# BichenWuUCB/squeezeDet

Hardware: NVIDIA H100
Metric: images/sec (1242x375, b=20) (higher is better)
Workload: dtype f32 (3xTF32 wgmma, fp32 accumulate)

## Files before the change

squeezedet_b200/csrc/conv_tc.cu:

```cuda
#include <cuda.h>
#include <cuda_runtime.h>
#include <stdint.h>
#include <stdlib.h>
#include <string.h>

#include <vector>

#include "common.cuh"
#include "conv_tc.cuh"

namespace sqdet {
namespace {

constexpr int TILE_M = 128;
constexpr int NUM_THREADS = 256;
constexpr int STAGES = 3;
constexpr int MAX_CHUNKS = 32;
constexpr int FT_W = 16, FQ_W = FT_W + 2, FQ_P = 10 * FQ_W;

enum TcMode { TC_ROWS, TC_GATHER, TC_HALO, TC_FIRE };

struct TcChunk {
  int ksize, pad_t, pad_l;
  int nk;
  int ncount;
  int y_off;
  int p_off;
  long long w_off;
};

struct TcParams {
  CUtensorMap amap, amap1;
  const float* x;
  float* y;
  const float* w;
  const float* bias;
  const float* scale;
  const float* shift;
  int B, H, W, Cin, Ho, Wo, stride, relu, y_cstride;
  long long M;
  int tiles_w, tiles_h;
  int nchunks;
  TcChunk chunks[MAX_CHUNKS];
};

__device__ __forceinline__ uint32_t smem_u32(const void* p) {
  return static_cast<uint32_t>(__cvta_generic_to_shared(p));
}
__device__ __forceinline__ void cp_async4(uint32_t dst, const void* src, bool valid) {
  asm volatile("cp.async.ca.shared.global [%0], [%1], 4, %2;" ::"r"(dst), "l"(src),
               "r"(valid ? 4 : 0)
               : "memory");
}
__device__ __forceinline__ void cp_async_arrive(uint64_t* bar) {
  asm volatile("cp.async.mbarrier.arrive.noinc.shared::cta.b64 [%0];" ::"r"(smem_u32(bar)) : "memory");
}

__device__ __forceinline__ void mbar_init(uint64_t* bar, int count) {
  asm volatile("mbarrier.init.shared::cta.b64 [%0], %1;" ::"r"(smem_u32(bar)), "r"(count) : "memory");
}
__device__ __forceinline__ void mbar_init_fence() {
  asm volatile("fence.mbarrier_init.release.cluster;\n\tfence.proxy.async.shared::cta;" ::: "memory");
}
__device__ __forceinline__ void mbar_arrive(uint64_t* bar) {
  asm volatile("mbarrier.arrive.shared::cta.b64 _, [%0];" ::"r"(smem_u32(bar)) : "memory");
}
__device__ __forceinline__ void mbar_expect_tx(uint64_t* bar, uint32_t bytes) {
  asm volatile("mbarrier.arrive.expect_tx.shared::cta.b64 _, [%0], %1;" ::"r"(smem_u32(bar)),
               "r"(bytes)
               : "memory");
}
__device__ __forceinline__ void mbar_wait(uint64_t* bar, uint32_t parity) {
  asm volatile(
      "{\n\t.reg .pred done;\n\t"
      "WAIT_%=:\n\t"
      "mbarrier.try_wait.parity.shared::cta.b64 done, [%0], %1;\n\t"
      "@!done bra WAIT_%=;\n\t}" ::"r"(smem_u32(bar)),
      "r"(parity)
      : "memory");
}

__device__ __forceinline__ void ring_init(uint64_t* full, uint64_t* empty, int full_count) {
  for (int s = 0; s < STAGES; ++s) {
    mbar_init(&full[s], full_count);
    mbar_init(&empty[s], NUM_THREADS / 32);
  }
  mbar_init_fence();
}
__device__ __forceinline__ int ring_acquire(uint64_t* empty, int j) {
  const int s = j % STAGES;
  if (j >= STAGES) mbar_wait(&empty[s], (j / STAGES & 1) ^ 1);
  return s;
}
__device__ __forceinline__ int ring_wait_full(uint64_t* full, int j) {
  const int s = j % STAGES;
  mbar_wait(&full[s], j / STAGES & 1);
  return s;
}
__device__ __forceinline__ void ring_release(uint64_t* empty, int j) {
  __syncwarp();
  if ((threadIdx.x & 31) == 0) mbar_arrive(&empty[j % STAGES]);
}

__device__ __forceinline__ void bulk_load(uint32_t dst, const void* src, uint32_t bytes, uint64_t* bar) {
  asm volatile(
      "cp.async.bulk.shared::cluster.global.mbarrier::complete_tx::bytes [%0], [%1], %2, [%3];" ::"r"(dst),
      "l"(src), "r"(bytes), "r"(smem_u32(bar))
      : "memory");
}
__device__ __forceinline__ void tma_load(uint32_t dst, const CUtensorMap* map, int c0, int c1, uint64_t* bar) {
  asm volatile(
      "cp.async.bulk.tensor.2d.shared::cluster.global.tile.mbarrier::complete_tx::bytes "
      "[%0], [%1, {%2, %3}], [%4];" ::"r"(dst),
      "l"(map), "r"(c0), "r"(c1), "r"(smem_u32(bar))
      : "memory");
}
__device__ __forceinline__ void tma_load(uint32_t dst, const CUtensorMap* map, int c0, int c1, int c2,
                                         int c3, uint64_t* bar) {
  asm volatile(
      "cp.async.bulk.tensor.4d.shared::cluster.global.tile.mbarrier::complete_tx::bytes "
      "[%0], [%1, {%2, %3, %4, %5}], [%6];" ::"r"(dst),
      "l"(map), "r"(c0), "r"(c1), "r"(c2), "r"(c3), "r"(smem_u32(bar))
      : "memory");
}
__device__ __forceinline__ void cluster_sync() {
  asm volatile("barrier.cluster.arrive.release.aligned;\n\tbarrier.cluster.wait.acquire.aligned;" ::: "memory");
}
__device__ __forceinline__ float4 ld_cluster_f4(uint32_t addr, int rank) {
  float4 v;
  asm volatile(
      "{\n\t.reg .b32 ra;\n\t"
      "mapa.shared::cluster.u32 ra, %4, %5;\n\t"
      "ld.shared::cluster.v4.f32 {%0, %1, %2, %3}, [ra];\n\t}"
      : "=f"(v.x), "=f"(v.y), "=f"(v.z), "=f"(v.w)
      : "r"(addr), "r"(rank)
      : "memory");
  return v;
}
__device__ __forceinline__ void wgmma_fence() { asm volatile("wgmma.fence.sync.aligned;" ::: "memory"); }
__device__ __forceinline__ void wgmma_commit() {
  asm volatile("wgmma.commit_group.sync.aligned;" ::: "memory");
}
template <int N>
__device__ __forceinline__ void wgmma_wait() {
  asm volatile("wgmma.wait_group.sync.aligned %0;" ::"n"(N) : "memory");
}
__device__ __forceinline__ void fence_operand(float& r) { asm volatile("" : "+f"(r)::"memory"); }
__device__ __forceinline__ void fence_operand(uint32_t& r) { asm volatile("" : "+r"(r)::"memory"); }

__device__ __forceinline__ uint64_t make_desc(uint32_t addr, uint32_t sbo) {
  return (uint64_t)((addr & 0x3FFFFu) >> 4) | ((uint64_t)(128 >> 4) << 16) |
         ((uint64_t)(sbo >> 4) << 32);
}

__device__ __forceinline__ float rn_tf32(float x) {
  return __uint_as_float((__float_as_uint(x) + 0x1000u) & 0xFFFFE000u);
}

template <int N>
struct Mma;
template <>
struct Mma<16> {
  static __device__ __forceinline__ void run(float (&d)[8], const uint32_t (&a)[4], uint64_t b,
                                             int acc) {
    asm volatile(
        "{\n\t.reg .pred p;\n\tsetp.ne.b32 p, %13, 0;\n\t"
        "wgmma.mma_async.sync.aligned.m64n16k8.f32.tf32.tf32 "
        "{%0, %1, %2, %3, %4, %5, %6, %7}, {%8, %9, %10, %11}, %12, p, 1, 1;\n\t}"
        : "+f"(d[0]), "+f"(d[1]), "+f"(d[2]), "+f"(d[3]), "+f"(d[4]), "+f"(d[5]), "+f"(d[6]),
          "+f"(d[7])
        : "r"(a[0]), "r"(a[1]), "r"(a[2]), "r"(a[3]), "l"(b), "r"(acc));
  }
};
template <>
struct Mma<32> {
  static __device__ __forceinline__ void run(float (&d)[16], const uint32_t (&a)[4], uint64_t b,
                                             int acc) {
    asm volatile(
        "{\n\t.reg .pred p;\n\tsetp.ne.b32 p, %21, 0;\n\t"
        "wgmma.mma_async.sync.aligned.m64n32k8.f32.tf32.tf32 "
        "{%0, %1, %2, %3, %4, %5, %6, %7, %8, %9, %10, %11, %12, %13, %14, %15}, "
        "{%16, %17, %18, %19}, %20, p, 1, 1;\n\t}"
        : "+f"(d[0]), "+f"(d[1]), "+f"(d[2]), "+f"(d[3]), "+f"(d[4]), "+f"(d[5]), "+f"(d[6]),
          "+f"(d[7]), "+f"(d[8]), "+f"(d[9]), "+f"(d[10]), "+f"(d[11]), "+f"(d[12]), "+f"(d[13]),
          "+f"(d[14]), "+f"(d[15])
        : "r"(a[0]), "r"(a[1]), "r"(a[2]), "r"(a[3]), "l"(b), "r"(acc));
  }
};
template <>
struct Mma<64> {
  static __device__ __forceinline__ void run(float (&d)[32], const uint32_t (&a)[4], uint64_t b,
                                             int acc) {
    asm volatile(
        "{\n\t.reg .pred p;\n\tsetp.ne.b32 p, %37, 0;\n\t"
        "wgmma.mma_async.sync.aligned.m64n64k8.f32.tf32.tf32 "
        "{%0, %1, %2, %3, %4, %5, %6, %7, %8, %9, %10, %11, %12, %13, %14, %15, "
        "%16, %17, %18, %19, %20, %21, %22, %23, %24, %25, %26, %27, %28, %29, %30, %31}, "
        "{%32, %33, %34, %35}, %36, p, 1, 1;\n\t}"
        : "+f"(d[0]), "+f"(d[1]), "+f"(d[2]), "+f"(d[3]), "+f"(d[4]), "+f"(d[5]), "+f"(d[6]),
          "+f"(d[7]), "+f"(d[8]), "+f"(d[9]), "+f"(d[10]), "+f"(d[11]), "+f"(d[12]), "+f"(d[13]),
          "+f"(d[14]), "+f"(d[15]), "+f"(d[16]), "+f"(d[17]), "+f"(d[18]), "+f"(d[19]),
          "+f"(d[20]), "+f"(d[21]), "+f"(d[22]), "+f"(d[23]), "+f"(d[24]), "+f"(d[25]),
          "+f"(d[26]), "+f"(d[27]), "+f"(d[28]), "+f"(d[29]), "+f"(d[30]), "+f"(d[31])
        : "r"(a[0]), "r"(a[1]), "r"(a[2]), "r"(a[3]), "l"(b), "r"(acc));
  }
};
template <>
struct Mma<72> {
  static __device__ __forceinline__ void run(float (&d)[36], const uint32_t (&a)[4], uint64_t b,
                                             int acc) {
    asm volatile(
        "{\n\t.reg .pred p;\n\tsetp.ne.b32 p, %41, 0;\n\t"
        "wgmma.mma_async.sync.aligned.m64n72k8.f32.tf32.tf32 "
        "{%0, %1, %2, %3, %4, %5, %6, %7, %8, %9, %10, %11, %12, %13, %14, %15, "
        "%16, %17, %18, %19, %20, %21, %22, %23, %24, %25, %26, %27, %28, %29, %30, %31, "
        "%32, %33, %34, %35}, "
        "{%36, %37, %38, %39}, %40, p, 1, 1;\n\t}"
        : "+f"(d[0]), "+f"(d[1]), "+f"(d[2]), "+f"(d[3]), "+f"(d[4]), "+f"(d[5]), "+f"(d[6]),
          "+f"(d[7]), "+f"(d[8]), "+f"(d[9]), "+f"(d[10]), "+f"(d[11]), "+f"(d[12]), "+f"(d[13]),
          "+f"(d[14]), "+f"(d[15]), "+f"(d[16]), "+f"(d[17]), "+f"(d[18]), "+f"(d[19]),
          "+f"(d[20]), "+f"(d[21]), "+f"(d[22]), "+f"(d[23]), "+f"(d[24]), "+f"(d[25]),
          "+f"(d[26]), "+f"(d[27]), "+f"(d[28]), "+f"(d[29]), "+f"(d[30]), "+f"(d[31]),
          "+f"(d[32]), "+f"(d[33]), "+f"(d[34]), "+f"(d[35])
        : "r"(a[0]), "r"(a[1]), "r"(a[2]), "r"(a[3]), "l"(b), "r"(acc));
  }
};

__host__ __device__ constexpr int halo_rows(int KC) {
  return (FQ_P * KC * 4 + 1023) / 1024 * 1024 / (KC * 4);
}
static_assert(2 * halo_rows(16) <= STAGES * TILE_M && 2 * halo_rows(32) <= STAGES * TILE_M,
              "two halo tiles fit in the A ring");
constexpr size_t conv_smem_bytes(int NT, int KC) {
  return 1024 + (size_t)STAGES * (2 * NT * KC + TILE_M * KC) * sizeof(float) + 2 * STAGES * sizeof(uint64_t);
}

__device__ __forceinline__ void split(const float (&v)[4], uint32_t (&ahi)[4], uint32_t (&alo)[4]) {
#pragma unroll
  for (int i = 0; i < 4; ++i) {
    const float hi = rn_tf32(v[i]);
    ahi[i] = __float_as_uint(hi);
    alo[i] = __float_as_uint(rn_tf32(v[i] - hi));
  }
}

__device__ __forceinline__ void load_split(const float* a0, const float* a1, int ks, int t,
                                           uint32_t (&ahi)[4], uint32_t (&alo)[4]) {
  split({a0[ks * 8 + t], a1[ks * 8 + t], a0[ks * 8 + t + 4], a1[ks * 8 + t + 4]}, ahi, alo);
}

template <int KC>
__device__ __forceinline__ int swz(int p) {
  return KC == 32 ? (p & 7) : ((p >> 1) & 3);
}
template <int KC>
__device__ __forceinline__ void load_split_swz(const float* tile, int p, int ks, int t,
                                               uint32_t (&ahi)[4], uint32_t (&alo)[4]) {
  const float* a0 = tile + p * KC + t;
  const float* a1 = a0 + 8 * KC;
  const int j0 = (2 * ks ^ swz<KC>(p)) * 4, j1 = ((2 * ks + 1) ^ swz<KC>(p)) * 4;
  split({a0[j0], a1[j0], a0[j1], a1[j1]}, ahi, alo);
}

template <int NT, int KC>
__device__ __forceinline__ void mma_step(float (&acc)[NT / 2], const uint32_t (&ahi)[4],
                                         const uint32_t (&alo)[4], uint32_t bhi, int ks) {
  constexpr uint32_t SBO = (KC / 4) * 128;
  const uint32_t blo = bhi + NT * KC * 4;
  const uint64_t dhi = make_desc(bhi + ks * 256, SBO), dlo = make_desc(blo + ks * 256, SBO);
#pragma unroll
  for (int i = 0; i < NT / 2; ++i) fence_operand(acc[i]);
  wgmma_fence();
  Mma<NT>::run(acc, alo, dhi, 0);
  Mma<NT>::run(acc, ahi, dlo, 1);
  Mma<NT>::run(acc, ahi, dhi, 1);
  wgmma_commit();
}

template <int N>
__device__ __forceinline__ void flush(float (&acc)[N], float (&sum)[N], uint32_t (&ahi)[4],
                                      uint32_t (&alo)[4]) {
#pragma unroll
  for (int i = 0; i < 4; ++i) fence_operand(ahi[i]), fence_operand(alo[i]);
#pragma unroll
  for (int i = 0; i < N; ++i) {
    fence_operand(acc[i]);
    sum[i] += acc[i];
  }
}

template <int NT, int KC, bool PIPE = true, typename LoadA>
__device__ __forceinline__ void mma_chunk(LoadA load_a, uint32_t bhi, float (&acc)[2][NT / 2],
                                          float (&sum)[NT / 2]) {
  constexpr int KSTEPS = KC / 8;
  uint32_t ahi[2][4], alo[2][4];
  if constexpr (!PIPE) {
#pragma unroll
    for (int ks = 0; ks < KSTEPS; ++ks) {
      load_a(ks, ahi[0], alo[0]);
      mma_step<NT, KC>(acc[0], ahi[0], alo[0], bhi, ks);
      wgmma_wait<0>();
      flush(acc[0], sum, ahi[0], alo[0]);
    }
  } else {
#pragma unroll
    for (int ks = 0; ks < KSTEPS; ++ks) {
      const int cur = ks & 1;
      load_a(ks, ahi[cur], alo[cur]);
      mma_step<NT, KC>(acc[cur], ahi[cur], alo[cur], bhi, ks);
      if (ks > 0) {
        wgmma_wait<1>();
        flush(acc[cur ^ 1], sum, ahi[cur ^ 1], alo[cur ^ 1]);
      }
    }
    constexpr int last = (KSTEPS - 1) & 1;
    wgmma_wait<0>();
    flush(acc[last], sum, ahi[last], alo[last]);
  }
}

struct HaloTile {
  int n, oy0, ox0;
};
__device__ __forceinline__ HaloTile halo_tile(int tiles_w, int tiles_h) {
  const int tx = blockIdx.x % tiles_w, rest = blockIdx.x / tiles_w;
  return {rest / tiles_h, rest % tiles_h * 8, tx * FT_W};
}

__device__ __forceinline__ float finish(const TcParams& p, const TcChunk& ch, int c, float v) {
  if (p.bias) v += p.bias[ch.p_off + c];
  if (p.scale) v = v * p.scale[ch.p_off + c] + p.shift[ch.p_off + c];
  if (p.relu) v = fmaxf(v, 0.f);
  return v;
}

template <typename Value>
__device__ __forceinline__ void store_pair(float* yrow, int c, int ncount, bool pair, Value value) {
  if (pair && c + 1 < ncount) {
    *reinterpret_cast<float2*>(yrow + c) = make_float2(value(c), value(c + 1));
  } else {
    if (c < ncount) yrow[c] = value(c);
    if (c + 1 < ncount) yrow[c + 1] = value(c + 1);
  }
}
__device__ __forceinline__ bool rows_pair_aligned(const TcParams& p, const TcChunk& ch) {
  return ((p.y_cstride | ch.y_off) & 1) == 0 && (reinterpret_cast<uintptr_t>(p.y) & 7) == 0;
}

template <int NT, int KC, int MODE, bool KSPLIT = false>
__global__ void __launch_bounds__(NUM_THREADS, 2)
conv_tc_kernel(const __grid_constant__ TcParams p) {
  static_assert(!KSPLIT || MODE == TC_HALO, "the K split walks halo-mode channel chunks");
  constexpr int NACC = NT / 2;
  constexpr int WST = 2 * NT * KC;
  constexpr uint32_t W_BYTES = WST * 4, TILE_BYTES = TILE_M * KC * 4, HALO_BYTES = FQ_P * KC * 4;
  constexpr int HROWS = halo_rows(KC);
  extern __shared__ __align__(16) uint8_t smem_raw[];
  float* const smem = reinterpret_cast<float*>(smem_raw + ((1024 - (smem_u32(smem_raw) & 1023)) & 1023));
  float* const sa = smem + STAGES * WST;
  uint64_t* const full = reinterpret_cast<uint64_t*>(sa + STAGES * TILE_M * KC);
  uint64_t* const empty = full + STAGES;

  const TcChunk& ch = p.chunks[blockIdx.y];
  const int tid = threadIdx.x;
  const int wg = tid >> 7, wq = (tid >> 5) & 3, lane = tid & 31, g = lane >> 2, t = lane & 3;
  const float* wch = p.w + ch.w_off;
  int k0 = 0, nk = ch.nk;
  const int taps = ch.ksize * ch.ksize;
  if (KSPLIT) {
    const int nc = ch.nk / taps, S = gridDim.z, z = blockIdx.z;
    k0 = z * nc / S * taps;
    nk = (z + 1) * nc / S * taps - k0;
    wch += (size_t)k0 * WST;
  }

  if (tid == 0) ring_init(full, empty, MODE == TC_GATHER ? NUM_THREADS + 1 : 1);
  __syncthreads();

  const long long m0 = (long long)blockIdx.x * TILE_M;

  auto gather_stage = [&](int kk, int s) {
    const int lp = tid >> 1, lh = tid & 1;
    const long long lm = m0 + lp;
    const bool lvalid = lm < p.M;
    int ln = 0, liy0 = 0, lix0 = 0;
    if (lvalid) {
      const int hw = p.Ho * p.Wo;
      ln = (int)(lm / hw);
      const int r = (int)(lm - (long long)ln * hw);
      liy0 = (r / p.Wo) * p.stride - ch.pad_t;
      lix0 = (r % p.Wo) * p.stride - ch.pad_l;
    }
    const float* xn = p.x + (size_t)ln * p.H * p.W * p.Cin;
    float* const arow = sa + (s * TILE_M + lp) * KC;
#pragma unroll
    for (int j = 0; j < KC / 2; ++j) {
      const int col = lh * (KC / 2) + j, k = kk * KC + col;
      const int tap = k / p.Cin, c = k - tap * p.Cin;
      const int iy = liy0 + tap / ch.ksize, ix = lix0 + tap % ch.ksize;
      const bool ok = lvalid && tap < taps && iy >= 0 && iy < p.H && ix >= 0 && ix < p.W;
      cp_async4(smem_u32(arow + ((col >> 2 ^ swz<KC>(lp)) << 2) + (col & 3)),
                ok ? xn + ((iy * p.W + ix) * p.Cin + c) : p.x, ok);
    }
    cp_async_arrive(&full[s]);
  };

  auto load_stage = [&](int j) {
    if (MODE != TC_GATHER && tid != 0) return;
    const int s = ring_acquire(empty, j);
    if (MODE == TC_GATHER) gather_stage(j, s);
    if (tid != 0) return;
    uint32_t bytes = W_BYTES;
    if (MODE == TC_ROWS) {
      bytes += TILE_BYTES;
      mbar_expect_tx(&full[s], bytes);
      tma_load(smem_u32(sa + s * TILE_M * KC), &p.amap, j * KC, (int)m0, &full[s]);
    } else if (MODE == TC_HALO) {
      const HaloTile tl = halo_tile(p.tiles_w, p.tiles_h);
      if (taps == 1) {
        bytes += TILE_BYTES;
        mbar_expect_tx(&full[s], bytes);
        tma_load(smem_u32(sa + s * TILE_M * KC), &p.amap1, (k0 + j) * KC, tl.ox0, tl.oy0, tl.n, &full[s]);
      } else if (j % 9 == 0) {
        bytes += HALO_BYTES;
        mbar_expect_tx(&full[s], bytes);
        tma_load(smem_u32(sa + (j / 9 & 1) * HROWS * KC), &p.amap, (k0 + j) / 9 * KC, tl.ox0 - 1,
                 tl.oy0 - 1, tl.n, &full[s]);
      } else {
        mbar_expect_tx(&full[s], bytes);
      }
    } else {
      mbar_expect_tx(&full[s], bytes);
    }
    bulk_load(smem_u32(smem + s * WST), wch + (size_t)j * WST, W_BYTES, &full[s]);
  };

#pragma unroll 1
  for (int j = 0; j < STAGES - 1 && j < nk; ++j) load_stage(j);

  const int arow0 = wg * 64 + wq * 16 + g;
  const int r = wg * 4 + wq;
  float acc[2][NACC], sum[NACC];
#pragma unroll
  for (int i = 0; i < NACC; ++i) acc[0][i] = acc[1][i] = sum[i] = 0.f;

  for (int kk = 0; kk < nk; ++kk) {
    if (kk + STAGES - 1 < nk) load_stage(kk + STAGES - 1);
    const int s = ring_wait_full(full, kk);

    const float* tile = sa + s * TILE_M * KC;
    int prow = arow0;
    if (MODE == TC_HALO && taps > 1) {
      const int c = kk / 9, tap = kk - c * 9;
      tile = sa + (c & 1) * HROWS * KC;
      prow = (r + tap / 3) * FQ_W + g + tap % 3;
    }
    mma_chunk<NT, KC, NT != 72>(
        [&](int ks, uint32_t(&ahi)[4], uint32_t(&alo)[4]) { load_split_swz<KC>(tile, prow, ks, t, ahi, alo); },
        smem_u32(smem + s * WST), acc, sum);
    ring_release(empty, kk);
  }

  if constexpr (KSPLIT) {
    static_assert(TILE_M * NT <= STAGES * (WST + TILE_M * KC), "the partial tile fits in the ring");
    float* const part = smem;
    __syncthreads();
#pragma unroll
    for (int h = 0; h < 2; ++h)
#pragma unroll
      for (int j = 0; j < NT / 8; ++j)
        *reinterpret_cast<float2*>(part + (arow0 + 8 * h) * NT + 8 * j + 2 * t) =
            make_float2(sum[4 * j + 2 * h], sum[4 * j + 2 * h + 1]);
    cluster_sync();
    constexpr int G = TILE_M * NT / 4;
    const int S = gridDim.z, z = blockIdx.z;
    const HaloTile tl = halo_tile(p.tiles_w, p.tiles_h);
    for (int i = z * G / S + tid; i < (z + 1) * G / S; i += NUM_THREADS) {
      const uint32_t at = smem_u32(part + 4 * i);
      float4 v = ld_cluster_f4(at, 0);
      for (int q = 1; q < S; ++q) {
        const float4 u = ld_cluster_f4(at, q);
        v.x += u.x, v.y += u.y, v.z += u.z, v.w += u.w;
      }
      const int px = 4 * i / NT, c0 = 4 * i % NT;
      const int oy = tl.oy0 + px / FT_W, ox = tl.ox0 + px % FT_W;
      if (oy >= p.Ho || ox >= p.Wo) continue;
      float* yrow = p.y + (((size_t)tl.n * p.Ho + oy) * p.Wo + ox) * p.y_cstride + ch.y_off;
      const float vs[4] = {v.x, v.y, v.z, v.w};
#pragma unroll
      for (int e = 0; e < 4; ++e)
        if (c0 + e < ch.ncount) yrow[c0 + e] = finish(p, ch, c0 + e, vs[e]);
    }
    cluster_sync();
  } else {
    const bool pair = rows_pair_aligned(p, ch);
#pragma unroll
    for (int h = 0; h < 2; ++h) {
      long long m = m0 + arow0 + 8 * h;
      if (MODE == TC_HALO) {
        const HaloTile tl = halo_tile(p.tiles_w, p.tiles_h);
        const int oy = tl.oy0 + r, ox = tl.ox0 + g + 8 * h;
        if (oy >= p.Ho || ox >= p.Wo) continue;
        m = ((long long)tl.n * p.Ho + oy) * p.Wo + ox;
      } else if (m >= p.M) {
        continue;
      }
      float* yrow = p.y + (size_t)m * p.y_cstride + ch.y_off;
#pragma unroll
      for (int j = 0; j < NT / 8; ++j)
        store_pair(yrow, 8 * j + 2 * t, ch.ncount, pair,
                   [&](int c) { return finish(p, ch, c, sum[4 * j + 2 * h + (c & 1)]); });
    }
  }
}

constexpr int FS = 16;
constexpr int FQ_ROWS = 192;

__host__ __device__ constexpr int fire_stage_floats(int KCI) { return 2 * FS * KCI + FQ_ROWS * KCI; }
constexpr size_t fire_smem_bytes(int KCI) {
  return 1024 + ((size_t)STAGES * fire_stage_floats(KCI) + FQ_ROWS * (FS + 4)) * sizeof(float) +
         2 * STAGES * sizeof(uint64_t);
}

template <int KCI>
__global__ void __launch_bounds__(NUM_THREADS, 2)
fire_tc_kernel(const __grid_constant__ TcParams p) {
  constexpr int QP = FS + 4;
  constexpr int SQW = 2 * FS * KCI;
  constexpr int STAGE = fire_stage_floats(KCI);
  constexpr uint32_t SQW_BYTES = SQW * 4, HALO_BYTES = FQ_P * KCI * 4, EX_BYTES = 2 * 64 * FS * 4;
  static_assert(EX_BYTES <= (SQW + FQ_P * KCI) * 4, "expand tile fits before the zeroed rows");
  static_assert(SQW_BYTES % 1024 == 0 && STAGE * 4 % 1024 == 0, "A tiles keep the swizzle's alignment");
  extern __shared__ __align__(16) uint8_t smem_raw[];
  float* const smem = reinterpret_cast<float*>(smem_raw + ((1024 - (smem_u32(smem_raw) & 1023)) & 1023));
  float* const q = smem + STAGES * STAGE;
  uint64_t* const full = reinterpret_cast<uint64_t*>(q + FQ_ROWS * QP);
  uint64_t* const empty = full + STAGES;

  const int tid = threadIdx.x;
  const int wg = tid >> 7, wq = (tid >> 5) & 3, lane = tid & 31, g = lane >> 2, t = lane & 3;
  const int nks = p.Cin / KCI;
  int total = 0;
#pragma unroll 1
  for (int c = 0; c < p.nchunks; ++c) total += p.chunks[c].nk;
  if (tid == 0) ring_init(full, empty, 1);
  for (int i = tid; i < STAGES * (FQ_ROWS - FQ_P) * KCI; i += NUM_THREADS) {
    const int s = i / ((FQ_ROWS - FQ_P) * KCI);
    smem[s * STAGE + SQW + FQ_P * KCI + i % ((FQ_ROWS - FQ_P) * KCI)] = 0.f;
  }
  __syncthreads();

  auto load_stage = [&](int j) {
    const int s = ring_acquire(empty, j);
    float* const st = smem + s * STAGE;
    if (j < nks) {
      const HaloTile tl = halo_tile(p.tiles_w, p.tiles_h);
      mbar_expect_tx(&full[s], SQW_BYTES + HALO_BYTES);
      tma_load(smem_u32(st + SQW), &p.amap, j * KCI, tl.ox0 - 1, tl.oy0 - 1, tl.n, &full[s]);
      bulk_load(smem_u32(st), p.w + (size_t)j * SQW, SQW_BYTES, &full[s]);
    } else {
      mbar_expect_tx(&full[s], EX_BYTES);
      bulk_load(smem_u32(st), p.w + (size_t)nks * SQW + (size_t)(j - nks) * 2 * 64 * FS, EX_BYTES,
                &full[s]);
    }
  };
  if (tid == 0) {
#pragma unroll 1
    for (int j = 0; j < STAGES - 1 && j < total; ++j) load_stage(j);
  }

  float accq[2][FS / 2], sq[2][FS / 2];
#pragma unroll
  for (int i = 0; i < FS / 2; ++i) accq[0][i] = accq[1][i] = sq[0][i] = sq[1][i] = 0.f;
  const int rb = wq * 16 + g;
  for (int kk = 0; kk < nks; ++kk) {
    if (tid == 0 && kk + STAGES - 1 < total) load_stage(kk + STAGES - 1);
    const float* st = smem + ring_wait_full(full, kk) * STAGE;
    const float* sa = st + SQW;
    if (wg == 0) {
      uint32_t qhi[2][4], qlo[2][4];
#pragma unroll
      for (int j = 0; j < 2 * (KCI / 8); ++j) {
        const int bi = j & 1, ks = j >> 1;
        load_split_swz<KCI>(sa, 128 * bi + rb, ks, t, qhi[bi], qlo[bi]);
        mma_step<FS, KCI>(accq[bi], qhi[bi], qlo[bi], smem_u32(st), ks);
        if (j > 0) {
          wgmma_wait<1>();
          flush(accq[bi ^ 1], sq[bi ^ 1], qhi[bi ^ 1], qlo[bi ^ 1]);
        }
      }
      wgmma_wait<0>();
      flush(accq[1], sq[1], qhi[1], qlo[1]);
    } else {
      mma_chunk<FS, KCI>(
          [&](int ks, uint32_t(&ahi)[4], uint32_t(&alo)[4]) {
            load_split_swz<KCI>(sa, 64 + rb, ks, t, ahi, alo);
          },
          smem_u32(st), accq, sq[0]);
    }
    ring_release(empty, kk);
  }
  {
    const HaloTile tl = halo_tile(p.tiles_w, p.tiles_h);
#pragma unroll
    for (int bi = 0; bi < 2; ++bi) {
      const int b = wg + 2 * bi;
      if (b >= 3) continue;
#pragma unroll
      for (int h = 0; h < 2; ++h) {
        const int row = b * 64 + wq * 16 + g + 8 * h;
        const int iy = tl.oy0 - 1 + row / FQ_W, ix = tl.ox0 - 1 + row % FQ_W;
        const bool ok = row < FQ_P && iy >= 0 && iy < p.H && ix >= 0 && ix < p.W;
#pragma unroll
        for (int j = 0; j < FS / 8; ++j)
#pragma unroll
          for (int e = 0; e < 2; ++e) {
            const int c = 8 * j + 2 * t + e;
            q[row * QP + c] = ok ? fmaxf(sq[bi][4 * j + 2 * h + e] + p.bias[c], 0.f) : 0.f;
          }
      }
    }
  }
  __syncthreads();

  const int r = wg * 4 + wq;
  float acc[2][32], sum[32];
#pragma unroll
  for (int i = 0; i < 32; ++i) acc[0][i] = acc[1][i] = sum[i] = 0.f;
  int c = 1, kk = 0;
  for (int j = nks; j < total; ++j) {
    if (tid == 0 && j + STAGES - 1 < total) load_stage(j + STAGES - 1);
    const int s = ring_wait_full(full, j);
    const TcChunk& ch = p.chunks[c];
    const int dy = ch.nk == 1 ? 1 : kk / 3, dx = ch.nk == 1 ? 1 : kk % 3;
    const int qr = (r + dy) * FQ_W + g + dx;
    mma_chunk<64, FS>(
        [&](int ks, uint32_t(&ahi)[4], uint32_t(&alo)[4]) {
          load_split(q + qr * QP, q + (qr + 8) * QP, ks, t, ahi, alo);
        },
        smem_u32(smem + s * STAGE), acc, sum);
    ring_release(empty, j);
    if (++kk == ch.nk) {
      const HaloTile tl = halo_tile(p.tiles_w, p.tiles_h);
      const int oy = tl.oy0 + r;
      const size_t prow = ((size_t)tl.n * p.H + oy) * p.W;
      const bool pair = rows_pair_aligned(p, ch);
#pragma unroll
      for (int h = 0; h < 2; ++h) {
        const int ox = tl.ox0 + g + 8 * h;
        if (oy >= p.H || ox >= p.W) continue;
        float* yrow = p.y + (prow + ox) * p.y_cstride + ch.y_off;
#pragma unroll
        for (int jn = 0; jn < 8; ++jn)
          store_pair(yrow, 8 * jn + 2 * t, ch.ncount, pair, [&](int col) {
            return fmaxf(sum[4 * jn + 2 * h + (col & 1)] + p.bias[ch.p_off + col], 0.f);
          });
      }
#pragma unroll
      for (int i = 0; i < 32; ++i) sum[i] = 0.f;
      kk = 0;
      ++c;
    }
  }
}

using TcKernel = void (*)(TcParams);

template <int KC, int MODE>
TcKernel conv_tc_instance(int NT) {
  return NT == 64 ? conv_tc_kernel<64, KC, MODE>
         : NT == 32 ? conv_tc_kernel<32, KC, MODE> : conv_tc_kernel<16, KC, MODE>;
}

TcKernel conv_tc_instance(int NT, int KC, int mode) {
  if (NT == 72) return mode == TC_HALO ? conv_tc_kernel<72, 32, TC_HALO> : conv_tc_kernel<72, 32, TC_ROWS>;
  if (mode == TC_GATHER) return conv_tc_instance<32, TC_GATHER>(NT);
  if (mode == TC_HALO)
    return KC == 32 ? conv_tc_instance<32, TC_HALO>(NT) : conv_tc_instance<16, TC_HALO>(NT);
  return KC == 32 ? conv_tc_instance<32, TC_ROWS>(NT) : conv_tc_instance<16, TC_ROWS>(NT);
}

struct PlanGroup {
  ConvGroup conv;
  int NT, KC, cin, chunk0;
};

}

struct TcImpl {
  TcParams prm{};
  int KC = 0;
  int mode = TC_ROWS;
  TcKernel kernel = nullptr;
  int ksplit = 1;
  size_t smem_bytes = 0;
  std::vector<PlanGroup> groups;
  int cout_total = 0;
  float* d_w = nullptr;
  float* d_bias = nullptr;
  float* d_scale = nullptr;
  float* d_shift = nullptr;
  long long w_floats = 0;
  const float* map_x = nullptr;
  int map_n = 0;
};

static inline float host_rn_tf32(float x) {
  uint32_t u;
  memcpy(&u, &x, 4);
  u = (u + 0x1000u) & 0xFFFFE000u;
  float r;
  memcpy(&r, &u, 4);
  return r;
}

static int pick_nt(const std::vector<ConvGroup>& groups, int KC, bool gather) {
  int best = 0;
  long long best_cost = 0;
  const bool head = !gather && KC == 32 && groups.size() == 1 && groups[0].Cout > 64 &&
                    groups[0].Cout <= 72;
  for (int nt : {72, 64, 32, 16}) {
    if (nt == 72 && !head) continue;
    long long chunks = 0;
    for (const auto& g : groups) chunks += (g.Cout + nt - 1) / nt;
    if (chunks > MAX_CHUNKS) continue;
    const long long cost = chunks * (nt + 32);
    if (!best || cost < best_cost) best = nt, best_cost = cost;
  }
  return best;
}

using EncodeTiledFn = CUresult (*)(CUtensorMap*, CUtensorMapDataType, cuuint32_t, void*, const cuuint64_t*,
                                   const cuuint64_t*, const cuuint32_t*, const cuuint32_t*,
                                   CUtensorMapInterleave, CUtensorMapSwizzle, CUtensorMapL2promotion,
                                   CUtensorMapFloatOOBfill);

static int encode_map(CUtensorMap* map, const float* x, int rank, const cuuint64_t* dims,
                      const cuuint32_t* box, int KC) {
  static EncodeTiledFn encode = [] {
    void* fn = nullptr;
    cudaDriverEntryPointQueryResult q;
    if (cudaGetDriverEntryPoint("cuTensorMapEncodeTiled", &fn, cudaEnableDefault, &q) != cudaSuccess ||
        q != cudaDriverEntryPointSuccess)
      fn = nullptr;
    return reinterpret_cast<EncodeTiledFn>(fn);
  }();
  if (!encode) return fail(SQDET_ERR_CUDA, "cuTensorMapEncodeTiled is not available from the driver");
  cuuint64_t strides[3];
  cuuint64_t stride = sizeof(float);
  for (int i = 0; i + 1 < rank; ++i) strides[i] = stride *= dims[i];
  const cuuint32_t elem_strides[4] = {1, 1, 1, 1};
  const CUresult rc = encode(map, CU_TENSOR_MAP_DATA_TYPE_FLOAT32, rank, const_cast<float*>(x), dims, strides,
                             box, elem_strides, CU_TENSOR_MAP_INTERLEAVE_NONE,
                             KC == 32 ? CU_TENSOR_MAP_SWIZZLE_128B : CU_TENSOR_MAP_SWIZZLE_64B,
                             CU_TENSOR_MAP_L2_PROMOTION_L2_128B, CU_TENSOR_MAP_FLOAT_OOB_FILL_NONE);
  if (rc != CUDA_SUCCESS)
    return fail(SQDET_ERR_CUDA, "cuTensorMapEncodeTiled failed (error " + std::to_string((int)rc) + ")");
  return SQDET_OK;
}

static int encode_nhwc_map(CUtensorMap* map, const float* x, int n, int H, int W, int C, int KC,
                           int box_w, int box_h) {
  const cuuint64_t dims[4] = {(cuuint64_t)C, (cuuint64_t)W, (cuuint64_t)H, (cuuint64_t)n};
  const cuuint32_t box[4] = {(cuuint32_t)KC, (cuuint32_t)box_w, (cuuint32_t)box_h, 1};
  return encode_map(map, x, 4, dims, box, KC);
}

static int update_maps(TcImpl* im, const float* x, int n) {
  if (im->mode == TC_GATHER || (im->map_x == x && im->map_n == n)) return SQDET_OK;
  TcParams& p = im->prm;
  im->map_x = nullptr;
  int rc;
  if (im->mode == TC_ROWS) {
    const cuuint64_t dims[2] = {(cuuint64_t)p.Cin, (cuuint64_t)n * p.H * p.W};
    const cuuint32_t box[2] = {(cuuint32_t)im->KC, TILE_M};
    rc = encode_map(&p.amap, x, 2, dims, box, im->KC);
  } else {
    rc = encode_nhwc_map(&p.amap, x, n, p.H, p.W, p.Cin, im->KC, FQ_W, 10);
    if (!rc && im->mode == TC_HALO) rc = encode_nhwc_map(&p.amap1, x, n, p.H, p.W, p.Cin, im->KC, FT_W, 8);
  }
  if (rc) return rc;
  im->map_x = x;
  im->map_n = n;
  return SQDET_OK;
}

static long long grid_blocks(const TcImpl* im, int n) {
  const TcParams& p = im->prm;
  if (im->mode == TC_HALO || im->mode == TC_FIRE) return (long long)n * p.tiles_h * p.tiles_w;
  return ((long long)n * p.Ho * p.Wo + TILE_M - 1) / TILE_M;
}

static int plan_common(TcImpl* im, int B, int H, int W, int Cin, int Ho, int Wo, int stride,
                       int pad_t, int pad_l, int relu, bool has_affine, int y_cstride) {
  const bool gather = im->mode == TC_GATHER;
  TcParams& p = im->prm;
  p.B = B; p.H = H; p.W = W; p.Cin = Cin; p.Ho = Ho; p.Wo = Wo; p.stride = stride;
  p.relu = relu; p.y_cstride = y_cstride; p.M = (long long)B * Ho * Wo;
  p.tiles_w = (Wo + FT_W - 1) / FT_W; p.tiles_h = (Ho + 7) / 8;
  if (p.M <= 0 || grid_blocks(im, B) > 0x7fffffffLL) return 0;
  std::vector<int> poffs;
  int poff = 0;
  for (const auto& g : im->groups) poffs.push_back(poff), poff += g.conv.Cout;
  std::vector<size_t> order;
  for (int pass = 0; pass < 2; ++pass)
    for (size_t gi = 0; gi < im->groups.size(); ++gi)
      if ((im->mode == TC_HALO && im->groups[gi].conv.ksize == 3) == (pass == 0)) order.push_back(gi);
  int nch = 0;
  long long woff = 0;
  for (const size_t gi : order) {
    PlanGroup& g = im->groups[gi];
    g.chunk0 = nch;
    const int taps = g.conv.ksize * g.conv.ksize;
    const int nk = gather ? (taps * g.cin + g.KC - 1) / g.KC : taps * (g.cin / g.KC);
    for (int cb = 0; cb < g.conv.Cout; cb += g.NT, ++nch) {
      TcChunk& c = p.chunks[nch];
      c.ksize = g.conv.ksize;
      c.pad_t = gather ? pad_t : g.conv.ksize / 2;
      c.pad_l = gather ? pad_l : g.conv.ksize / 2;
      c.nk = nk;
      c.ncount = g.conv.Cout - cb < g.NT ? g.conv.Cout - cb : g.NT;
      c.y_off = g.conv.y_off + cb;
      c.p_off = poffs[gi] + cb;
      c.w_off = woff;
      woff += (long long)nk * 2 * g.NT * g.KC;
    }
  }
  p.nchunks = nch;
  im->cout_total = poff;
  im->w_floats = woff;
  cudaError_t ce = cudaFuncSetAttribute(im->kernel, cudaFuncAttributeMaxDynamicSharedMemorySize,
                                        (int)im->smem_bytes);
  if (ce != cudaSuccess) return cuda_fail(ce, "cudaFuncSetAttribute(tensor-core kernel)");
  SQ_CUDA(cudaMalloc(&im->d_w, sizeof(float) * (size_t)woff));
  SQ_CUDA(cudaMalloc(&im->d_bias, sizeof(float) * poff));
  SQ_CUDA(cudaMemset(im->d_bias, 0, sizeof(float) * poff));
  if (has_affine) {
    SQ_CUDA(cudaMalloc(&im->d_scale, sizeof(float) * poff));
    SQ_CUDA(cudaMalloc(&im->d_shift, sizeof(float) * poff));
  }
  p.w = im->d_w;
  p.bias = im->d_bias;
  p.scale = im->d_scale;
  p.shift = im->d_shift;
  return 1;
}

static void pack_tiles(const float* w, long long kreal, int cout, int n0, int NT, int KC, int nk,
                       int taps, int cin, float* dst) {
  for (int kk = 0; kk < nk; ++kk) {
    float* hi_t = dst + (size_t)kk * 2 * NT * KC;
    float* lo_t = hi_t + NT * KC;
    const long long k0 = (long long)(kk % taps) * cin + (long long)(kk / taps) * KC;
    for (int n = 0; n < NT; ++n)
      for (int k = 0; k < KC; ++k) {
        const long long kg = k0 + k;
        const float v = (n0 + n < cout && kg < kreal) ? w[kg * cout + n0 + n] : 0.f;
        const float hi = host_rn_tf32(v);
        const size_t at = ((size_t)(n / 8) * (KC / 4) + k / 4) * 32 + (n % 8) * 4 + k % 4;
        hi_t[at] = hi;
        lo_t[at] = host_rn_tf32(v - hi);
      }
  }
}

static void pack_group(const TcImpl* im, const PlanGroup& g, const float* w_hwio, std::vector<float>& packed) {
  const int taps = im->mode == TC_GATHER ? 1 : g.conv.ksize * g.conv.ksize;
  int ci = g.chunk0;
  for (int cb = 0; cb < g.conv.Cout; cb += g.NT, ++ci) {
    const TcChunk& c = im->prm.chunks[ci];
    pack_tiles(w_hwio, (long long)g.conv.ksize * g.conv.ksize * g.cin, g.conv.Cout, cb, g.NT, g.KC,
               c.nk, taps, g.cin, packed.data() + c.w_off);
  }
}

struct ClusterLaunch {
  cudaLaunchAttribute attr;
  cudaLaunchConfig_t cfg;
  ClusterLaunch(dim3 grid, size_t smem, int S, cudaStream_t stream) : attr{}, cfg{} {
    attr.id = cudaLaunchAttributeClusterDimension;
    attr.val.clusterDim.x = attr.val.clusterDim.y = 1;
    attr.val.clusterDim.z = (unsigned)S;
    cfg.gridDim = dim3(grid.x, grid.y, grid.z * S);
    cfg.blockDim = dim3(NUM_THREADS);
    cfg.dynamicSmemBytes = smem;
    cfg.stream = stream;
    cfg.attrs = &attr;
    cfg.numAttrs = 1;
  }
};

constexpr int MAX_KSPLIT = 4;
constexpr int MIN_RANK_CHUNKS = 4;

static int plan_ksplit(TcImpl* im, int forced) {
  const TcKernel split = conv_tc_kernel<72, 32, TC_HALO, true>;
  const int nc = im->prm.chunks[0].nk / 9;
  if (forced < 0 || forced > MAX_KSPLIT || forced > nc)
    return fail(SQDET_ERR_INVALID_ARG, "K split outside [1, min(4, channel chunks)]");
  SQ_CUDA(cudaFuncSetAttribute(split, cudaFuncAttributeMaxDynamicSharedMemorySize, (int)im->smem_bytes));
  int S = forced;
  if (!forced) {
    int dev = 0, sms = 0, per_sm = 0;
    SQ_CUDA(cudaGetDevice(&dev));
    SQ_CUDA(cudaDeviceGetAttribute(&sms, cudaDevAttrMultiProcessorCount, dev));
    SQ_CUDA(cudaOccupancyMaxActiveBlocksPerMultiprocessor(&per_sm, im->kernel, NUM_THREADS, im->smem_bytes));
    const long long ctas = grid_blocks(im, im->prm.B) * im->prm.nchunks;
    S = 1;
    long long best_waves = (ctas + per_sm * sms - 1) / (per_sm * sms);
    for (int s = 2; s <= MAX_KSPLIT && s * MIN_RANK_CHUNKS <= nc; ++s) {
      int clusters = 0;
      const ClusterLaunch l(dim3(1), im->smem_bytes, s, nullptr);
      SQ_CUDA(cudaOccupancyMaxActiveClusters(&clusters, split, &l.cfg));
      if (clusters < 1) continue;
      const long long waves = (ctas + clusters - 1) / clusters;
      if (waves * S < best_waves * s) S = s, best_waves = waves;
    }
  }
  if (S > 1) im->kernel = split;
  im->ksplit = S;
  return 1;
}

bool tc_conv_eligible(int Cin, int Cout, int size, int stride, int padding) {
  if (stride != 1 || padding != SQDET_PAD_SAME || (size != 1 && size != 3)) return false;
  return Cin % 16 == 0 && Cin >= 16 && Cout > 0;
}

int tc_conv_plan(TcConvPlan* plan, int B, int H, int W, int Cin, const std::vector<ConvGroup>& convs,
                 int stride, int padding, int relu, bool has_affine, int y_cstride, int k_split) {
  plan->impl = nullptr;
  const int size = convs[0].ksize;
  const bool gather = convs.size() == 1 && Cin == 3 && size == 3 && (stride == 1 || stride == 2) &&
                      convs[0].Cout > 0;
  if (!gather)
    for (const auto& g : convs)
      if (!tc_conv_eligible(Cin, g.Cout, g.ksize, stride, padding)) return 0;
  const Geom gh = tf_geometry(H, size, stride, padding);
  const Geom gw = tf_geometry(W, size, stride, padding);
  if (gh.out <= 0 || gw.out <= 0) return 0;
  const int KC = (gather || Cin % 32 == 0) ? 32 : 16;
  const int NT = pick_nt(convs, KC, gather);
  if (!NT) return 0;
  int mode = gather ? TC_GATHER : TC_ROWS;
  for (const auto& g : convs)
    if (!gather && g.ksize == 3) mode = TC_HALO;
  TcImpl* im = plan->impl = new TcImpl();
  im->KC = KC;
  im->mode = mode;
  im->kernel = conv_tc_instance(NT, KC, mode);
  im->smem_bytes = conv_smem_bytes(NT, KC);
  for (const auto& g : convs) im->groups.push_back({g, NT, KC, Cin, 0});
  int rc = plan_common(im, B, H, W, Cin, gh.out, gw.out, stride, gh.pad_before, gw.pad_before,
                       relu, has_affine, y_cstride);
  if (rc > 0 && NT == 72 && mode == TC_HALO) {
    rc = plan_ksplit(im, k_split);
  } else if (rc > 0 && k_split > 1) {
    rc = fail(SQDET_ERR_INVALID_ARG, "a K split needs a 72-wide 3x3 tensor-core plan");
  }
  if (rc <= 0) tc_conv_release(plan);
  return rc;
}

int tc_conv_k_split(const TcConvPlan& plan) { return plan.impl ? plan.impl->ksplit : 1; }

int tc_fire_plan(TcConvPlan* plan, int B, int H, int W, int Cin, int S, int E1, int E3) {
  plan->impl = nullptr;
  if (Cin % 16 || Cin < 16 || S != FS || E1 <= 0 || E3 <= 0) return 0;
  if ((E1 + 63) / 64 + (E3 + 63) / 64 > 16) return 0;
  const int KCI = Cin % 32 == 0 ? 32 : 16;
  TcImpl* im = plan->impl = new TcImpl();
  im->KC = KCI;
  im->mode = TC_FIRE;
  im->kernel = KCI == 32 ? fire_tc_kernel<32> : fire_tc_kernel<16>;
  im->smem_bytes = fire_smem_bytes(KCI);
  im->groups = {{{1, FS, 0}, FS, KCI, Cin, 0}, {{1, E1, 0}, 64, FS, FS, 0}, {{3, E3, E1}, 64, FS, FS, 0}};
  const int rc = plan_common(im, B, H, W, Cin, H, W, 1, 0, 0, 1, false, E1 + E3);
  if (rc <= 0) tc_conv_release(plan);
  return rc;
}

int tc_conv_pack_weights(TcConvPlan* plan, const std::vector<const float*>& w_hwio,
                         const std::vector<const float*>& bias) {
  TcImpl* im = plan->impl;
  std::vector<float> packed((size_t)im->w_floats, 0.f);
  for (size_t gi = 0; gi < im->groups.size(); ++gi) pack_group(im, im->groups[gi], w_hwio[gi], packed);
  SQ_CUDA(cudaMemcpy(im->d_w, packed.data(), packed.size() * sizeof(float), cudaMemcpyHostToDevice));
  int off = 0;
  for (size_t gi = 0; gi < im->groups.size(); ++gi) {
    const int n = im->groups[gi].conv.Cout;
    if (bias[gi]) SQ_CUDA(cudaMemcpy(im->d_bias + off, bias[gi], sizeof(float) * n, cudaMemcpyHostToDevice));
    off += n;
  }
  return SQDET_OK;
}

int tc_conv_set_affine(TcConvPlan* plan, const float* scale, const float* shift) {
  TcImpl* im = plan->impl;
  if (!im->d_scale) return fail(SQDET_ERR_STATE, "tc conv planned without an affine epilogue");
  SQ_CUDA(cudaMemcpy(im->d_scale, scale, sizeof(float) * im->cout_total, cudaMemcpyHostToDevice));
  SQ_CUDA(cudaMemcpy(im->d_shift, shift, sizeof(float) * im->cout_total, cudaMemcpyHostToDevice));
  return SQDET_OK;
}

int launch_conv_tc(const TcConvPlan& plan, const float* x_dev, float* y_dev, int n,
                   cudaStream_t stream) {
  TcImpl* im = plan.impl;
  if (n < 1 || n > im->prm.B) return fail(SQDET_ERR_INVALID_ARG, "launch_conv_tc: image count outside [1, B]");
  const int rc = update_maps(im, x_dev, n);
  if (rc) return rc;
  TcParams prm = im->prm;
  prm.x = x_dev;
  prm.y = y_dev;
  prm.B = n;
  prm.M = (long long)n * prm.Ho * prm.Wo;
  const dim3 grid((unsigned)grid_blocks(im, n), im->mode == TC_FIRE ? 1u : (unsigned)prm.nchunks);
  if (im->ksplit > 1) {
    const ClusterLaunch l(grid, im->smem_bytes, im->ksplit, stream);
    SQ_CUDA(cudaLaunchKernelEx(&l.cfg, im->kernel, prm));
  } else {
    im->kernel<<<grid, NUM_THREADS, im->smem_bytes, stream>>>(prm);
  }
  SQ_CHECK_LAUNCH(im->mode == TC_FIRE ? "fire_tc_kernel" : "conv_tc_kernel");
  return SQDET_OK;
}

void tc_conv_release(TcConvPlan* plan) {
  TcImpl* im = plan->impl;
  if (!im) return;
  cudaFree(im->d_w);
  cudaFree(im->d_bias);
  cudaFree(im->d_scale);
  cudaFree(im->d_shift);
  delete im;
  plan->impl = nullptr;
}

int tc_conv_oneshot(TcConvPlan* plan, const std::vector<const float*>& w_hwio_dev,
                    const std::vector<const float*>& bias_dev, const float* scale_dev,
                    const float* shift_dev, const float* x_dev, float* y_dev, cudaStream_t stream) {
  TcImpl* im = plan->impl;
  if (!im) return 1;
  const size_t ng = im->groups.size();
  std::vector<std::vector<float>> w(ng), b(ng);
  std::vector<float> sc, sh;
  std::vector<const float*> w_host(ng), b_host(ng);
  cudaError_t ce = cudaSuccess;
  auto download = [&ce](std::vector<float>& dst, const float* src, size_t n) {
    dst.resize(n);
    if (ce == cudaSuccess) ce = cudaMemcpy(dst.data(), src, n * sizeof(float), cudaMemcpyDeviceToHost);
    return dst.data();
  };
  for (size_t gi = 0; gi < ng; ++gi) {
    const ConvGroup& g = im->groups[gi].conv;
    w_host[gi] = download(w[gi], w_hwio_dev[gi], (size_t)g.ksize * g.ksize * im->groups[gi].cin * g.Cout);
    b_host[gi] = bias_dev[gi] ? download(b[gi], bias_dev[gi], g.Cout) : nullptr;
  }
  if (scale_dev) download(sc, scale_dev, im->cout_total), download(sh, shift_dev, im->cout_total);
  int rc = ce == cudaSuccess ? tc_conv_pack_weights(plan, w_host, b_host)
                             : cuda_fail(ce, "tc_conv_oneshot: parameter download");
  if (!rc && scale_dev) rc = tc_conv_set_affine(plan, sc.data(), sh.data());
  if (!rc) rc = launch_conv_tc(*plan, x_dev, y_dev, im->prm.B, stream);
  ce = cudaStreamSynchronize(stream);
  tc_conv_release(plan);
  if (rc) return rc;
  if (ce != cudaSuccess) return cuda_fail(ce, "tc_conv_oneshot sync");
  return SQDET_OK;
}

}
```

Measured before the change: 4820.

## Pack two 3x3 taps per pipeline stage in halo and fire-expand kernels

For halo-mode convolutions with 16-channel chunks and for the fire expand phase, each ring stage now holds the weights for two taps instead of one. The per-stage barrier waits, releases and bulk-load issues drop to roughly half, and each stage runs longer back-to-back wgmma chains. In exchange the weight buffer per stage doubles, which raises shared memory use and may lower occupancy. It also adds index bookkeeping for a trailing single-tap stage.

```diff
diff --git a/squeezedet_b200/csrc/conv_tc.cu b/squeezedet_b200/csrc/conv_tc.cu
--- a/squeezedet_b200/csrc/conv_tc.cu
+++ b/squeezedet_b200/csrc/conv_tc.cu
@@ -231,8 +231,10 @@
 }
 static_assert(2 * halo_rows(16) <= STAGES * TILE_M && 2 * halo_rows(32) <= STAGES * TILE_M,
               "two halo tiles fit in the A ring");
-constexpr size_t conv_smem_bytes(int NT, int KC) {
-  return 1024 + (size_t)STAGES * (2 * NT * KC + TILE_M * KC) * sizeof(float) + 2 * STAGES * sizeof(uint64_t);
+__host__ __device__ constexpr int conv_tps(int KC, int MODE) { return MODE == TC_HALO && KC == 16 ? 2 : 1; }
+constexpr size_t conv_smem_bytes(int NT, int KC, int MODE) {
+  return 1024 + (size_t)STAGES * (conv_tps(KC, MODE) * 2 * NT * KC + TILE_M * KC) * sizeof(float) +
+         2 * STAGES * sizeof(uint64_t);
 }
 
 __device__ __forceinline__ void split(const float (&v)[4], uint32_t (&ahi)[4], uint32_t (&alo)[4]) {
@@ -289,31 +291,32 @@
   }
 }
 
-template <int NT, int KC, bool PIPE = true, typename LoadA>
+template <int NT, int KC, int TILES = 1, bool PIPE = true, typename LoadA>
 __device__ __forceinline__ void mma_chunk(LoadA load_a, uint32_t bhi, float (&acc)[2][NT / 2],
                                           float (&sum)[NT / 2]) {
-  constexpr int KSTEPS = KC / 8;
+  constexpr int KSTEPS = KC / 8, STEPS = TILES * KSTEPS;
+  constexpr uint32_t TILE_BYTES = 2 * NT * KC * sizeof(float);
   uint32_t ahi[2][4], alo[2][4];
   if constexpr (!PIPE) {
 #pragma unroll
-    for (int ks = 0; ks < KSTEPS; ++ks) {
+    for (int ks = 0; ks < STEPS; ++ks) {
       load_a(ks, ahi[0], alo[0]);
-      mma_step<NT, KC>(acc[0], ahi[0], alo[0], bhi, ks);
+      mma_step<NT, KC>(acc[0], ahi[0], alo[0], bhi + ks / KSTEPS * TILE_BYTES, ks % KSTEPS);
       wgmma_wait<0>();
       flush(acc[0], sum, ahi[0], alo[0]);
     }
   } else {
 #pragma unroll
-    for (int ks = 0; ks < KSTEPS; ++ks) {
+    for (int ks = 0; ks < STEPS; ++ks) {
       const int cur = ks & 1;
       load_a(ks, ahi[cur], alo[cur]);
-      mma_step<NT, KC>(acc[cur], ahi[cur], alo[cur], bhi, ks);
+      mma_step<NT, KC>(acc[cur], ahi[cur], alo[cur], bhi + ks / KSTEPS * TILE_BYTES, ks % KSTEPS);
       if (ks > 0) {
         wgmma_wait<1>();
         flush(acc[cur ^ 1], sum, ahi[cur ^ 1], alo[cur ^ 1]);
       }
     }
-    constexpr int last = (KSTEPS - 1) & 1;
+    constexpr int last = (STEPS - 1) & 1;
     wgmma_wait<0>();
     flush(acc[last], sum, ahi[last], alo[last]);
   }
@@ -352,12 +355,16 @@
 conv_tc_kernel(const __grid_constant__ TcParams p) {
   static_assert(!KSPLIT || MODE == TC_HALO, "the K split walks halo-mode channel chunks");
   constexpr int NACC = NT / 2;
+  constexpr int TPS = conv_tps(KC, MODE);
+  constexpr int SPC = (9 + TPS - 1) / TPS;
   constexpr int WST = 2 * NT * KC;
+  constexpr int SW = TPS * WST;
   constexpr uint32_t W_BYTES = WST * 4, TILE_BYTES = TILE_M * KC * 4, HALO_BYTES = FQ_P * KC * 4;
   constexpr int HROWS = halo_rows(KC);
+  static_assert(STAGES <= SPC + 1, "a halo buffer's last step is released before its next load");
   extern __shared__ __align__(16) uint8_t smem_raw[];
   float* const smem = reinterpret_cast<float*>(smem_raw + ((1024 - (smem_u32(smem_raw) & 1023)) & 1023));
-  float* const sa = smem + STAGES * WST;
+  float* const sa = smem + STAGES * SW;
   uint64_t* const full = reinterpret_cast<uint64_t*>(sa + STAGES * TILE_M * KC);
   uint64_t* const empty = full + STAGES;
 
@@ -373,6 +380,7 @@
     nk = (z + 1) * nc / S * taps - k0;
     wch += (size_t)k0 * WST;
   }
+  const int nsteps = TPS > 1 && taps > 1 ? nk / 9 * SPC : nk;
 
   if (tid == 0) ring_init(full, empty, MODE == TC_GATHER ? NUM_THREADS + 1 : 1);
   __syncthreads();
@@ -410,7 +418,13 @@
     const int s = ring_acquire(empty, j);
     if (MODE == TC_GATHER) gather_stage(j, s);
     if (tid != 0) return;
-    uint32_t bytes = W_BYTES;
+    int k = j, nt = 1;
+    if (TPS > 1 && taps > 1) {
+      const int c = j / SPC, tap0 = (j - c * SPC) * TPS;
+      k = c * 9 + tap0;
+      nt = 9 - tap0 < TPS ? 9 - tap0 : TPS;
+    }
+    uint32_t bytes = nt * W_BYTES;
     if (MODE == TC_ROWS) {
       bytes += TILE_BYTES;
       mbar_expect_tx(&full[s], bytes);
@@ -421,10 +435,10 @@
         bytes += TILE_BYTES;
         mbar_expect_tx(&full[s], bytes);
         tma_load(smem_u32(sa + s * TILE_M * KC), &p.amap1, (k0 + j) * KC, tl.ox0, tl.oy0, tl.n, &full[s]);
-      } else if (j % 9 == 0) {
+      } else if (k % 9 == 0) {
         bytes += HALO_BYTES;
         mbar_expect_tx(&full[s], bytes);
-        tma_load(smem_u32(sa + (j / 9 & 1) * HROWS * KC), &p.amap, (k0 + j) / 9 * KC, tl.ox0 - 1,
+        tma_load(smem_u32(sa + (k / 9 & 1) * HROWS * KC), &p.amap, (k0 + k) / 9 * KC, tl.ox0 - 1,
                  tl.oy0 - 1, tl.n, &full[s]);
       } else {
         mbar_expect_tx(&full[s], bytes);
@@ -432,11 +446,11 @@
     } else {
       mbar_expect_tx(&full[s], bytes);
     }
-    bulk_load(smem_u32(smem + s * WST), wch + (size_t)j * WST, W_BYTES, &full[s]);
+    bulk_load(smem_u32(smem + s * SW), wch + (size_t)k * WST, nt * W_BYTES, &full[s]);
   };
 
 #pragma unroll 1
-  for (int j = 0; j < STAGES - 1 && j < nk; ++j) load_stage(j);
+  for (int j = 0; j < STAGES - 1 && j < nsteps; ++j) load_stage(j);
 
   const int arow0 = wg * 64 + wq * 16 + g;
   const int r = wg * 4 + wq;
@@ -444,25 +458,36 @@
 #pragma unroll
   for (int i = 0; i < NACC; ++i) acc[0][i] = acc[1][i] = sum[i] = 0.f;
 
-  for (int kk = 0; kk < nk; ++kk) {
-    if (kk + STAGES - 1 < nk) load_stage(kk + STAGES - 1);
+  for (int kk = 0; kk < nsteps; ++kk) {
+    if (kk + STAGES - 1 < nsteps) load_stage(kk + STAGES - 1);
     const int s = ring_wait_full(full, kk);
 
     const float* tile = sa + s * TILE_M * KC;
-    int prow = arow0;
+    int prow[TPS];
+    bool whole = true;
+#pragma unroll
+    for (int i = 0; i < TPS; ++i) prow[i] = arow0;
     if (MODE == TC_HALO && taps > 1) {
-      const int c = kk / 9, tap = kk - c * 9;
+      const int c = kk / SPC, tap0 = (kk - c * SPC) * TPS;
       tile = sa + (c & 1) * HROWS * KC;
-      prow = (r + tap / 3) * FQ_W + g + tap % 3;
-    }
-    mma_chunk<NT, KC, NT != 72>(
-        [&](int ks, uint32_t(&ahi)[4], uint32_t(&alo)[4]) { load_split_swz<KC>(tile, prow, ks, t, ahi, alo); },
-        smem_u32(smem + s * WST), acc, sum);
+#pragma unroll
+      for (int i = 0; i < TPS; ++i) prow[i] = (r + (tap0 + i) / 3) * FQ_W + g + (tap0 + i) % 3;
+      whole = tap0 + TPS <= 9;
+    } else {
+      whole = TPS == 1;
+    }
+    const auto load_a = [&](int ks, uint32_t(&ahi)[4], uint32_t(&alo)[4]) {
+      load_split_swz<KC>(tile, prow[ks / (KC / 8)], ks % (KC / 8), t, ahi, alo);
+    };
+    if (TPS == 1 || whole)
+      mma_chunk<NT, KC, TPS, NT != 72>(load_a, smem_u32(smem + s * SW), acc, sum);
+    else
+      mma_chunk<NT, KC, 1, NT != 72>(load_a, smem_u32(smem + s * SW), acc, sum);
     ring_release(empty, kk);
   }
 
   if constexpr (KSPLIT) {
-    static_assert(TILE_M * NT <= STAGES * (WST + TILE_M * KC), "the partial tile fits in the ring");
+    static_assert(TILE_M * NT <= STAGES * (SW + TILE_M * KC), "the partial tile fits in the ring");
     float* const part = smem;
     __syncthreads();
 #pragma unroll
@@ -517,7 +542,11 @@
 constexpr int FS = 16;
 constexpr int FQ_ROWS = 192;
 
-__host__ __device__ constexpr int fire_stage_floats(int KCI) { return 2 * FS * KCI + FQ_ROWS * KCI; }
+constexpr int FIRE_TPS = 2;
+__host__ __device__ constexpr int fire_stage_floats(int KCI) {
+  return ((2 * FS * KCI + FQ_ROWS * KCI > FIRE_TPS * 2 * 64 * FS ? 2 * FS * KCI + FQ_ROWS * KCI
+                                                                  : FIRE_TPS * 2 * 64 * FS) + 255) & ~255;
+}
 constexpr size_t fire_smem_bytes(int KCI) {
   return 1024 + ((size_t)STAGES * fire_stage_floats(KCI) + FQ_ROWS * (FS + 4)) * sizeof(float) +
          2 * STAGES * sizeof(uint64_t);
@@ -529,8 +558,8 @@
   constexpr int QP = FS + 4;
   constexpr int SQW = 2 * FS * KCI;
   constexpr int STAGE = fire_stage_floats(KCI);
-  constexpr uint32_t SQW_BYTES = SQW * 4, HALO_BYTES = FQ_P * KCI * 4, EX_BYTES = 2 * 64 * FS * 4;
-  static_assert(EX_BYTES <= (SQW + FQ_P * KCI) * 4, "expand tile fits before the zeroed rows");
+  constexpr int EXW = 2 * 64 * FS;
+  constexpr uint32_t SQW_BYTES = SQW * 4, HALO_BYTES = FQ_P * KCI * 4, EX_BYTES = EXW * 4;
   static_assert(SQW_BYTES % 1024 == 0 && STAGE * 4 % 1024 == 0, "A tiles keep the swizzle's alignment");
   extern __shared__ __align__(16) uint8_t smem_raw[];
   float* const smem = reinterpret_cast<float*>(smem_raw + ((1024 - (smem_u32(smem_raw) & 1023)) & 1023));
@@ -541,9 +570,9 @@
   const int tid = threadIdx.x;
   const int wg = tid >> 7, wq = (tid >> 5) & 3, lane = tid & 31, g = lane >> 2, t = lane & 3;
   const int nks = p.Cin / KCI;
-  int total = 0;
+  int total = nks;
 #pragma unroll 1
-  for (int c = 0; c < p.nchunks; ++c) total += p.chunks[c].nk;
+  for (int c = 1; c < p.nchunks; ++c) total += (p.chunks[c].nk + FIRE_TPS - 1) / FIRE_TPS;
   if (tid == 0) ring_init(full, empty, 1);
   for (int i = tid; i < STAGES * (FQ_ROWS - FQ_P) * KCI; i += NUM_THREADS) {
     const int s = i / ((FQ_ROWS - FQ_P) * KCI);
@@ -551,6 +580,7 @@
   }
   __syncthreads();
 
+  int lc = 1, lt = 0;
   auto load_stage = [&](int j) {
     const int s = ring_acquire(empty, j);
     float* const st = smem + s * STAGE;
@@ -560,9 +590,11 @@
       tma_load(smem_u32(st + SQW), &p.amap, j * KCI, tl.ox0 - 1, tl.oy0 - 1, tl.n, &full[s]);
       bulk_load(smem_u32(st), p.w + (size_t)j * SQW, SQW_BYTES, &full[s]);
     } else {
-      mbar_expect_tx(&full[s], EX_BYTES);
-      bulk_load(smem_u32(st), p.w + (size_t)nks * SQW + (size_t)(j - nks) * 2 * 64 * FS, EX_BYTES,
-                &full[s]);
+      const TcChunk& ch = p.chunks[lc];
+      const int n = ch.nk - lt < FIRE_TPS ? ch.nk - lt : FIRE_TPS;
+      mbar_expect_tx(&full[s], n * EX_BYTES);
+      bulk_load(smem_u32(st), p.w + ch.w_off + (size_t)lt * EXW, n * EX_BYTES, &full[s]);
+      if ((lt += n) == ch.nk) lt = 0, ++lc;
     }
   };
   if (tid == 0) {
@@ -633,15 +665,22 @@
     if (tid == 0 && j + STAGES - 1 < total) load_stage(j + STAGES - 1);
     const int s = ring_wait_full(full, j);
     const TcChunk& ch = p.chunks[c];
-    const int dy = ch.nk == 1 ? 1 : kk / 3, dx = ch.nk == 1 ? 1 : kk % 3;
-    const int qr = (r + dy) * FQ_W + g + dx;
-    mma_chunk<64, FS>(
-        [&](int ks, uint32_t(&ahi)[4], uint32_t(&alo)[4]) {
-          load_split(q + qr * QP, q + (qr + 8) * QP, ks, t, ahi, alo);
-        },
-        smem_u32(smem + s * STAGE), acc, sum);
+    int qr[FIRE_TPS];
+#pragma unroll
+    for (int i = 0; i < FIRE_TPS; ++i) {
+      const int dy = ch.nk == 1 ? 1 : (kk + i) / 3, dx = ch.nk == 1 ? 1 : (kk + i) % 3;
+      qr[i] = (r + dy) * FQ_W + g + dx;
+    }
+    const auto load_a = [&](int ks, uint32_t(&ahi)[4], uint32_t(&alo)[4]) {
+      const int qi = qr[ks / (FS / 8)];
+      load_split(q + qi * QP, q + (qi + 8) * QP, ks % (FS / 8), t, ahi, alo);
+    };
+    if (kk + FIRE_TPS <= ch.nk)
+      mma_chunk<64, FS, FIRE_TPS>(load_a, smem_u32(smem + s * STAGE), acc, sum);
+    else
+      mma_chunk<64, FS, 1>(load_a, smem_u32(smem + s * STAGE), acc, sum);
     ring_release(empty, j);
-    if (++kk == ch.nk) {
+    if ((kk += FIRE_TPS) >= ch.nk) {
       const HaloTile tl = halo_tile(p.tiles_w, p.tiles_h);
       const int oy = tl.oy0 + r;
       const size_t prow = ((size_t)tl.n * p.H + oy) * p.W;
@@ -950,7 +989,7 @@
   im->KC = KC;
   im->mode = mode;
   im->kernel = conv_tc_instance(NT, KC, mode);
-  im->smem_bytes = conv_smem_bytes(NT, KC);
+  im->smem_bytes = conv_smem_bytes(NT, KC, mode);
   for (const auto& g : convs) im->groups.push_back({g, NT, KC, Cin, 0});
   int rc = plan_common(im, B, H, W, Cin, gh.out, gw.out, stride, gh.pad_before, gw.pad_before,
                        relu, has_affine, y_cstride);
```

Result: no change. 4867, median of 6 (+1.0%).
